# ansonb/RECON

Measured on AMD Instinct MI355X. Metric: edges aggregated/sec (GAT fwd+bwd) on synthetic KG-context graphs, higher is better.
Workload: dtype f32

## Files before the change

### recon_amd/csrc/gat_atp.hip

```cpp
#include <math.h>
#include <stdlib.h>
#include "recon_common.h"

#include <type_traits>

namespace recon {
namespace {

constexpr int kBlock = 256;

__device__ __forceinline__ int xcd_block(int b, int nb) {
    const int q = nb >> 3, r = nb & 7, x = b & 7, i = b >> 3;
    return (x < r ? x * (q + 1) : r * (q + 1) + (x - r) * q) + i;
}
template <int VEC, bool B16>
__device__ __forceinline__ void load_in(float (&r)[VEC], const float* base, int64_t e) {
    if constexpr (!B16) {
        load_vec<VEC>(r, base + e);
    } else {
        const uint16_t* b = reinterpret_cast<const uint16_t*>(base) + e;
        if constexpr (VEC == 4) {
            const uint2 t = *reinterpret_cast<const uint2*>(b);
            r[0] = __builtin_bit_cast(float, t.x << 16); r[1] = __builtin_bit_cast(float, t.x & 0xffff0000u);
            r[2] = __builtin_bit_cast(float, t.y << 16); r[3] = __builtin_bit_cast(float, t.y & 0xffff0000u);
// ... 45 lines not shown
        float t = 0.f;
#pragma unroll
        for (int g = 0; g < 16; ++g) t += red[g][c];
        u[static_cast<int64_t>(h) * W + w] = t;
    }
    if (aux) {
        __syncthreads();
        red[grp][c] = mx;
        __syncthreads();
        if (threadIdx.x < 64) {
            float m = 0.f;
#pragma unroll
            for (int g = 0; g < 16; ++g) m = fmaxf(m, red[g][threadIdx.x]);
#pragma unroll
            for (int off = 32; off > 0; off >>= 1) m = fmaxf(m, __shfl_xor(m, off, 64));
            const int b = blockIdx.y * gridDim.x + blockIdx.x;
            if (threadIdx.x == 0) aux[hx2_blkmax_word(b)] = __builtin_bit_cast(uint32_t, m);
        }
        const int nblk = gridDim.x * gridDim.y, b = blockIdx.y * gridDim.x + blockIdx.x;
        const int total = static_cast<int>(kHx2AuxBytes / 4) - kHx2QuantityWords;
        const int per_b = (total + nblk - 1) / nblk;
        for (int i = b * per_b + threadIdx.x; i < min(total, (b + 1) * per_b); i += 1024) aux[kHx2QuantityWords + i] = 0u;
    }
}

__global__ void __launch_bounds__(256) k_score_vec_bwd(const float* __restrict__ a, const float* __restrict__ a2,
                                                       const float* __restrict__ gu, int32_t D, int32_t W, float* __restrict__ ga,
                                                       float* __restrict__ ga2, uint32_t* __restrict__ rezero, int32_t rezero_words) {
    __shared__ float red[256];
    const int d = blockIdx.x, h = blockIdx.y;
    if (rezero && d == 0 && h == 0)
        for (int i = threadIdx.x; i < rezero_words; i += 256) rezero[i] = 0u;
    const int64_t row = (static_cast<int64_t>(h) * D + d) * W;
    const float a2v = a2[h * D + d];
    float s = 0.f;
    for (int w = threadIdx.x; w < W; w += 256) {
        const float g = gu[static_cast<int64_t>(h) * W + w];
        s = fmaf(a[row + w], g, s);
        if (ga) ga[row + w] += a2v * g;
    }
    red[threadIdx.x] = s;
    __syncthreads();
    for (int off = 128; off > 0; off >>= 1) {
        if (threadIdx.x < off) red[threadIdx.x] += red[threadIdx.x + off];
        __syncthreads();
    }
    if (threadIdx.x == 0 && ga2) ga2[h * D + d] = red[0];
}

__global__ void __launch_bounds__(256) k_atp_weights_finish(const float* __restrict__ partial, int32_t splits, int32_t W, int32_t D, int32_t H,
                                                            const float* __restrict__ a, const float* __restrict__ a2,
                                                            const float* __restrict__ gu, float* __restrict__ ga, float* __restrict__ ga2,
                                                            uint32_t* __restrict__ rezero, int32_t rezero_words) {
    __shared__ float tile[32][33];
    if (rezero && blockIdx.x == 0)
        for (int i = threadIdx.x; i < rezero_words; i += 256) rezero[i] = 0u;
    const int tw = (W + 31) / 32, td = (D + 31) / 32, ntile = tw * td * H;
    if (static_cast<int>(blockIdx.x) < ntile) {
        const int b = blockIdx.x, h = b / (td * tw), m0 = ((b / td) % tw) * 32, n0 = (b % td) * 32;
        const int tx = threadIdx.x & 31, ty = threadIdx.x >> 5;
        const int64_t MN = static_cast<int64_t>(W) * D;
        const float* pz = partial + static_cast<int64_t>(h) * splits * MN;
        float acc[4] = {0.f, 0.f, 0.f, 0.f};
        int64_t off[4];
        bool ok[4];
#pragma unroll
        for (int i = 0; i < 4; ++i) {
            const int m = m0 + ty + 8 * i, n = n0 + tx;
            ok[i] = m < W && n < D;
            off[i] = ok[i] ? static_cast<int64_t>(m) * D + n : 0;
        }
        for (int z = 0; z < splits; ++z) {
#pragma unroll
            for (int i = 0; i < 4; ++i) acc[i] += pz[z * MN + off[i]];
        }
#pragma unroll
        for (int i = 0; i < 4; ++i) tile[ty + 8 * i][tx] = ok[i] ? acc[i] : 0.f;
        __syncthreads();
#pragma unroll
        for (int i = 0; i < 4; ++i) {
            const int n = n0 + ty + 8 * i, m = m0 + tx;
            if (m < W && n < D)
                ga[(static_cast<int64_t>(h) * D + n) * W + m] = fmaf(a2[h * D + n], gu[static_cast<int64_t>(h) * W + m], tile[tx][ty + 8 * i]);
        }
    } else if (ga2) {
        const int lane = threadIdx.x & 63, wave = threadIdx.x >> 6;
        const int r0 = (static_cast<int>(blockIdx.x) - ntile) * 8 + wave * 2;
#pragma unroll
        for (int i = 0; i < 2; ++i) {
            const int r = r0 + i;
            if (r >= H * D) break;
            const int h = r / D;
            float sum = 0.f;
            for (int w = 4 * lane; w < W; w += 256) {
                const float4 av = *reinterpret_cast<const float4*>(a + static_cast<int64_t>(r) * W + w);
                const float4 gv = *reinterpret_cast<const float4*>(gu + static_cast<int64_t>(h) * W + w);
                sum = fmaf(av.x, gv.x, fmaf(av.y, gv.y, fmaf(av.z, gv.z, fmaf(av.w, gv.w, sum))));
            }
#pragma unroll
            for (int off = 32; off > 0; off >>= 1) sum += __shfl_xor(sum, off, 64);
            if (lane == 0) ga2[r] = sum;
        }
    }
}

__global__ void __launch_bounds__(256) k_elu_grad_q(const float* __restrict__ gy, int32_t ld_gy, const float* __restrict__ y,
                                                    int32_t ld_y, int32_t N, int32_t H, int32_t D, int32_t concat,
                                                    float* __restrict__ gh, float* __restrict__ q, uint16_t* __restrict__ ghp,
                                                    int64_t ld_p, int64_t plane_p, int32_t f16x2, const Hx2Scale gsc,
                                                    float* __restrict__ row_inv, int64_t row_inv_ld, uint32_t* __restrict__ amax_q,
                                                    const int32_t* __restrict__ row_node) {
    constexpr int IPW = 4;
    const int lane = threadIdx.x & 63;
    const int item0 = (blockIdx.x * 4 + (threadIdx.x >> 6)) * IPW;
    const int total = N * H;
    if (item0 >= total) return;
    const bool v4 = ((D | ld_gy | ld_y) & 3) == 0;
    if (v4 && D <= 256) {
        const int c = 4 * lane;
        const bool cok = c < D;
        const int cc = cok ? c : 0;
        float4 g4[IPW], y4[IPW];
#pragma unroll
        for (int j = 0; j < IPW; ++j) {
            const int it = min(item0 + j, total - 1);
            const int node = it / H, h = it % H;
            g4[j] = *reinterpret_cast<const float4*>(gy + static_cast<int64_t>(row_node ? row_node[node] : node) * ld_gy + h * D + cc);
            y4[j] = *reinterpret_cast<const float4*>(y + static_cast<int64_t>(node) * ld_y + h * D + cc);
        }
        const float gs_t = (f16x2 && !row_inv) ? hx2_scale_wave(gsc) : 1.f;
        float ov[IPW][4], pv[IPW], rmx[IPW];
#pragma unroll
        for (int j = 0; j < IPW; ++j) {
            const float gv[4] = {g4[j].x, g4[j].y, g4[j].z, g4[j].w}, yv[4] = {y4[j].x, y4[j].y, y4[j].z, y4[j].w};
            float part = 0.f, mx = 0.f;
#pragma unroll
// ... 1770 lines not shown
    const int n = blockIdx.x * (kBlock / 64) + __builtin_amdgcn_readfirstlane(threadIdx.x >> 6);
    if (n >= N) return;
    const int r = node_row[n];
    float* o = out + static_cast<int64_t>(n) * ld_out;
    const float* in = rows + static_cast<int64_t>(r < 0 ? 0 : r) * ld_rows;
    if (vec4) {
        for (int c = 4 * lane; c < width; c += 256) {
            const float4 v = r >= 0 ? *reinterpret_cast<const float4*>(in + c) : make_float4(0.f, 0.f, 0.f, 0.f);
            *reinterpret_cast<float4*>(o + c) = v;
        }
    } else {
        for (int c = lane; c < width; c += 64) o[c] = r >= 0 ? in[c] : 0.f;
    }
}
}
extern "C" int recon_rows_expand(const float* rows, int32_t ld_rows, const int32_t* node_row, int32_t N, int32_t width, float* out, int32_t ld_out,
                                 recon_stream_t stream) {
    if (N < 0 || width < 0 || ld_rows < width || ld_out < width || (N > 0 && (!node_row || !out)) || (N > 0 && width > 0 && !rows)) return RECON_ERR_INVALID;
    if (N == 0 || width == 0) return RECON_OK;
    const int vec4 = ((width | ld_rows | ld_out) & 3) == 0 && !((reinterpret_cast<uintptr_t>(rows) | reinterpret_cast<uintptr_t>(out)) & 15);
    hipLaunchKernelGGL(k_rows_expand, dim3(static_cast<unsigned>(ceil_div64(N, kBlock / 64))), dim3(kBlock), 0, as_stream(stream), rows, ld_rows, node_row, N, width, out,
                       ld_out, vec4);
    RECON_CHECK_LAUNCH();
    return RECON_OK;
}

extern "C" int recon_gat_atp_fwd(const recon_graph* g, const recon_gat_atp_args* a, recon_stream_t stream) {
    int rc = recon_gat_atp_scores(g, a, stream);
    if (rc != RECON_OK) return rc;
    rc = recon_gat_atp_aggregate(g, a, stream);
    if (rc != RECON_OK) return rc;
    return recon_gat_atp_project(g, a, stream);
}

extern "C" int recon_gat_atp_bwd_gee_bf16_supported(int32_t F, int32_t R, int32_t D, int32_t H) {
    recon::AtpShape s;
    if (!recon_gat_atp_bf16_io_supported(F, R, D, H) || !recon::atp_shape(F, R, H, &s)) return 0;
    const size_t lds_k2 = static_cast<size_t>(H) * (F + R) * sizeof(float) + (kBlock / 64) * 512;
    const bool lring = s.vec == 4 && s.kr == 1 && lds_k2 + (kBlock / 64) * kK2LdsRingBytes <= 64 * 1024 && cfg_char(CFG_K2_LDS_RING) != '0';
    return (s.ht >= H && lring) ? 1 : 0;
}

extern "C" size_t recon_gat_atp_bwd_split_bytes(int32_t N, int32_t D, int32_t H) {
    if (N <= 0 || D <= 0 || H <= 0) return 256;
    return align_up(static_cast<size_t>(3) * N * bx3_kp(H * D) * 2, 256);
}

extern "C" size_t recon_gat_atp_bwd_partial_floats(int32_t N, int32_t E, int32_t F, int32_t R, int32_t D, int32_t H) {
    const int64_t W = 2LL * F + R;
    int s1 = gemm_pick_split_k(static_cast<int32_t>(W), D, N, H);
    const int s2 = bx3_kmajor_splits(N, bx3_kmajor_split_k(static_cast<int32_t>(W), D, N, H));
    if (s2 > s1) s1 = s2;
    size_t need = static_cast<size_t>(s1) * H * D * W;
    (void)E; (void)F; (void)R;
    return need > 0 ? need : 1;
}

constexpr int kSkinnySlices = 1024;
constexpr size_t kSkinnySrcLdsMax = 32 * 1024;
static int skinny_rpb(int64_t rows) {
    const int rpb = static_cast<int>(ceil_div64(rows, kSkinnySlices));
    return rpb < 32 ? 32 : rpb;
}
extern "C" size_t recon_gat_atp_bwd_partial2_floats(int32_t N, int32_t E, int32_t F, int32_t R, int32_t D, int32_t H) {
    (void)N; (void)E; (void)D; (void)H;
    const size_t mx = static_cast<size_t>(F > R ? F : R);
    return static_cast<size_t>(3) * kSkinnySlices * 16 * mx;
}

extern "C" int recon_gat_atp_bwd(const recon_graph* g, const recon_gat_atp_bwd_args* b, recon_stream_t stream) {
    return recon_gat_atp_bwd_phase(g, b, RECON_ATP_BWD_ALL, stream);
}

extern "C" int recon_gat_atp_bwd_phase(const recon_graph* g, const recon_gat_atp_bwd_args* b, int32_t phases, recon_stream_t stream) {
    if (!b) return RECON_ERR_INVALID;
    const recon_gat_atp_args* a = &b->fwd;
    int rc = check_atp(g, a);
    if (rc != RECON_OK) return rc;
    if (!recon_gat_atp_supported(a->N, a->E, a->F, a->R, a->D, a->H)) return RECON_ERR_UNSUPPORTED;
    if (!a->Z || !a->Zk || !b->grad_out || !b->g_V || !b->gxd || !b->Gs || !b->g_u || !b->partial || !b->partial2 || !b->q) return RECON_ERR_INVALID;
    if (a->E > 0 && (!a->sigma || !b->g_sigma || !b->Gxs)) return RECON_ERR_INVALID;
    const bool hx2 = atp_hx2(a);
    if ((a->concat || atp_rows(g, a).row_node) && !b->g_h && !hx2) return RECON_ERR_INVALID;
    if (hx2 && (!b->gh_split || (reinterpret_cast<uintptr_t>(b->gh_split) & 15) || (b->ld_gout & 3))) return RECON_ERR_INVALID;
    if (b->ld_gout < a->H * a->D) return RECON_ERR_INVALID;
    if (a->N == 0) return RECON_OK;
    hipStream_t st = as_stream(stream);
    const int32_t N = a->N, E = a->E, F = a->F, R = a->R, D = a->D, H = a->H, W = 2 * F + R;
    const AtpRows rw = atp_rows(g, a);
    const int32_t NR = rw.n;
    const int64_t HD = 1LL * H * D;
    AtpShape s;
    atp_shape(F, R, H, &s);
    const size_t lds_u = static_cast<size_t>(H) * (F + R) * sizeof(float);
    if (lds_u > 60 * 1024) return RECON_ERR_UNSUPPORTED;
    const size_t lds_k2 = lds_u + (kBlock / 64) * 512;

    const float* gh = b->grad_out;
    int32_t ld_gh = b->ld_gout;
    const int64_t ld_ghp = bx3_kp(static_cast<int32_t>(HD));
    const bool gh_planes = hx2 || (b->gh_split && a->a_split && !(reinterpret_cast<uintptr_t>(b->gh_split) & 15) && (D % 8) == 0 &&
                                   ((b->ld_gout | a->ld_out) & 3) == 0);
    uint16_t* ghp = gh_planes ? static_cast<uint16_t*>(b->gh_split) : nullptr;
    const int64_t ldi = (static_cast<int64_t>(NR) + 7) / 8 * 8;
    const size_t inv_off = align_up(static_cast<size_t>(2) * N * bx3_kp(static_cast<int32_t>(HD)) * 2, 256);
    const bool row_scaled = hx2 && D <= 256 && ((a->ld_out | b->ld_gout) & 3) == 0 && cfg_char(CFG_ATP_ROW_SCALE) != '0' &&
                            inv_off + static_cast<size_t>(H) * ldi * sizeof(float) <= recon_gat_atp_bwd_split_bytes(N, D, H);
// ... 110 lines not shown
                nb_total = 0;
                for (int i = 0; i < 3; ++i) {
                    sj[i] = SkinnyJob{nullptr, nullptr, nullptr, nullptr, 0, 0, 0, 0, 1, 0};
                    rj[i] = SkinnyRedJob{nullptr, nullptr, 0, 0, 0, 0, 0, 1, 0};
                    if (i >= count) continue;
                    const Prod& q = pr[i];
                    if (q.rows <= 0) {
                        for (int j = 0; j < q.nj; ++j) (void)hipMemsetAsync(q.out + (j % q.P) * q.S1 + (j / q.P) * q.S2, 0, sizeof(float) * q.K, st);
                        continue;
                    }
                    const int rpb = skinny_rpb(q.rows);
                    const int nb = static_cast<int>(ceil_div64(q.rows, rpb));
                    float* part = b->partial2 + i * third;
                    sj[i] = SkinnyJob{q.G, q.X, q.gather, part, q.ldg, q.nj, q.rows, q.K, rpb, nb};
                    rj[i] = SkinnyRedJob{part, q.out, q.S1, q.S2, nb, q.nj, q.K, q.P, static_cast<int32_t>(ceil_div64(1LL * q.nj * q.K, 16))};
                    if (q.nj > nj_max) nj_max = q.nj;
                    nb_total += nb; nr_total += rj[i].nblocks;
                }
                if (share) { launch_src(); if (nb_total == 0) return; }
                else {
                    if (nb_total == 0) return;
                    const dim3 gp(static_cast<unsigned>(nb_total));
                    if (a->io_bf16) {
                        if (nj_max <= 8) hipLaunchKernelGGL((k_skinny_tn_partial<8, true>), gp, dim3(256), 0, st, sj[0], sj[1], sj[2]);
                        else hipLaunchKernelGGL((k_skinny_tn_partial<16, true>), gp, dim3(256), 0, st, sj[0], sj[1], sj[2]);
                    } else if (nj_max <= 8) hipLaunchKernelGGL((k_skinny_tn_partial<8>), gp, dim3(256), 0, st, sj[0], sj[1], sj[2]);
                    else hipLaunchKernelGGL((k_skinny_tn_partial<16>), gp, dim3(256), 0, st, sj[0], sj[1], sj[2]);
                }
                hipLaunchKernelGGL(k_skinny_reduce, dim3(static_cast<unsigned>(nr_total)), dim3(1024), 0, st, rj[0], rj[1], rj[2]);
            };
            if (H <= 8) {
                const Prod pr[3] = {{b->Gs, 2 * H, H, a->x, rw.row_node, NR, F, H, W, 0, b->g_u},
                                    {b->Gs + H, 2 * H, H, a->x, nullptr, N, F, H, W, 0, b->g_u + F},
                                    {b->g_sigma, H, H, a->edge_embed, ee_gather, E, R, H, W, 0, b->g_u + 2 * F}};
                run_jobs(pr, 3);
            } else {
                for (int j = 0; j < 2 * H; ++j) {
                    const Prod one = {b->Gs + j, 2 * H, 1, a->x, j < H ? rw.row_node : nullptr, j < H ? NR : N, F, 1, W, 0,
                                      b->g_u + static_cast<int64_t>(j % H) * W + (j / H) * F};
                    run_jobs(&one, 1);
                }
                for (int h0 = 0; h0 < H; h0 += 16) {
                    const int nh = H - h0 < 16 ? H - h0 : 16;
                    const Prod one = {b->g_sigma + h0, H, nh, a->edge_embed, ee_gather, E, R, nh, W, 0, b->g_u + static_cast<int64_t>(h0) * W + 2 * F};
                    run_jobs(&one, 1);
                }
            }
        }
        RECON_CHECK_LAUNCH();
    }
    }
    if (b->g_a || b->g_a_2) {
        if (!b->g_a) return RECON_ERR_INVALID;
        if (phases & RECON_ATP_BWD_WEIGHTS) {
            OperandDesc A = plain_operand(a->V, static_cast<int64_t>(H) * W);
            OperandDesc B = plain_operand(gh, ld_gh);
            OutputDesc C = plain_output(b->g_a, W);
            GemmBatch bw = bt;
            bw.a_bs = W; bw.b_bs = D; bw.c_bs = static_cast<int64_t>(D) * W; bw.c_transpose = 1;
            const int64_t ldv = static_cast<int64_t>(H) * W;
            if (hx2) {
                const int sk = bx3_kmajor_splits(NR, bx3_kmajor_split_k(W, D, NR, H));
                rc = gemm_hx2_kmajor_batched(W, D, NR, a->V, 2LL * W, W, 2LL * NR * W, b->gh_split, 2LL * D, D, 2LL * NR * D,
                                             H, sk, b->partial, static_cast<const char*>(a->aux) + kHx2ZeroPageOffset, atp_scale_v(a), atp_scale_g(a), st,
                                             atp_dst_shared(a), row_inv, ldi);
                if (rc == RECON_OK && (phases & RECON_ATP_BWD_EARLY_SUM)) rc = splitk_reduce(b->partial, sk, W, D, C, bw.c_bs, H, 0, true, st);
            } else if (gh_planes && bx3_kmajor_supported(a->V, ldv, W, ld_ghp, D, W, D)) {
                const int sk = bx3_kmajor_splits(NR, bx3_kmajor_split_k(W, D, NR, H));
                rc = gemm_bx3_kmajor_batched(W, D, NR, a->V, ldv, W, b->gh_split, ld_ghp, static_cast<int64_t>(NR) * ld_ghp, D, H, sk, b->partial, st);
                if (rc == RECON_OK) rc = splitk_reduce(b->partial, sk, W, D, C, bw.c_bs, H, 0, true, st);
            } else {
                const int sk = gemm_pick_split_k(W, D, NR, H);
                rc = gemm_f32_batched(W, D, NR, A, false, B, false, C, bw, sk, b->partial, st);
            }
            if (rc != RECON_OK) return rc;
        }
        if ((phases & RECON_ATP_BWD_FINISH) && hx2 && !(phases & RECON_ATP_BWD_EARLY_SUM)) {
            const int sk = bx3_kmajor_splits(NR, bx3_kmajor_split_k(W, D, NR, H));
            const int ntile = static_cast<int>(ceil_div64(W, 32) * ceil_div64(D, 32)) * H;
            hipLaunchKernelGGL(k_atp_weights_finish, dim3(static_cast<unsigned>(ntile + ceil_div64(1LL * H * D, 8))), dim3(256), 0, st, b->partial, sk, W,
                               D, H, a->a, a->a_2, b->g_u, b->g_a, b->g_a_2, atp_q(a, 3), kHx2QuantityWords);
        } else if (phases & RECON_ATP_BWD_FINISH)
        hipLaunchKernelGGL(k_score_vec_bwd, dim3(static_cast<unsigned>(D), static_cast<unsigned>(H)), dim3(256), 0, st, a->a, a->a_2, b->g_u,
                           D, W, b->g_a, b->g_a_2, atp_hx2(a) ? atp_q(a, 3) : nullptr, kHx2QuantityWords);
        RECON_CHECK_LAUNCH();
    } else if ((phases & RECON_ATP_BWD_FINISH) && atp_hx2(a)) {
        if (hipMemsetAsync(atp_q(a, 3), 0, sizeof(uint32_t) * kHx2QuantityWords, st) != hipSuccess) return RECON_ERR_LAUNCH;
    }
    return RECON_OK;
}
```

### recon_amd/csrc/gemm_hx2.hip

```cpp
#include <stdlib.h>
#include "gemm_tile16.h"

namespace recon {
namespace {

constexpr int T = 2;

struct Hx2Args {
    const _Float16* Ap; const _Float16* Bp;
    int64_t a_plane, a_row, a_bs;
    int64_t b_plane, b_row, b_bs;
    OutputDesc C;
    int64_t c_bs;
    int32_t M, N, K;
    int32_t epilogue, c_vec4, xcd_remap, c_plain;
    int32_t a_shared_k;
    Hx2Scale sa, sb;
    const float* row_inv; int64_t row_inv_bs;
    int32_t a_span_bytes;
};

struct Hx2Terms {
    using V = f16x8;
    static constexpr int T = 2, NP = 3;
// ... 198 lines not shown
#pragma unroll
        for (int g = 0; g < (TN + 1) / 2; ++g) {
            if (2 * g + 2 < TN) read_pair(2 * g + 2, b[(g + 1) & 1]);
            __builtin_amdgcn_sched_barrier(0);
            if (2 * g + 1 < TN) products<Hx2Terms, 2>(acc, af, b[g & 1], 2 * g);
            else products<Hx2Terms, 1>(acc, af, b[g & 1], 2 * g);
            __builtin_amdgcn_sched_barrier(0);
            if (g == 0) {
                dma_b(kt + 1, (kt + 1) & 1);
                load_a(anext2, kt + 2);
                __builtin_amdgcn_sched_barrier(0);
            }
        }
    };

    dma_b(0, 0);
    load_a(araw[0], 0);
    load_a(araw[1], 1);
    const float ia = hx2_inv(hx2_scale_wave(p.sa)), ib = hx2_inv(hx2_scale_wave(p.sb));
    int kt = 0;
#pragma unroll 1
    for (; kt + 3 <= KT; kt += 3) {
        step(kt, araw[0], araw[2]);
        step(kt + 1, araw[1], araw[0]);
        step(kt + 2, araw[2], araw[1]);
    }
    if (kt < KT) step(kt, araw[0], araw[2]);
    if (kt + 1 < KT) step(kt + 1, araw[1], araw[0]);
    (void)Kp;
    dma_wait<0>();
    float rsc[2][4];
#pragma unroll
    for (int i = 0; i < 2; ++i)
#pragma unroll
        for (int r = 0; r < 4; ++r)
            rsc[i][r] = (p.row_inv ? p.row_inv[bz * p.row_inv_bs + min(m0 + mb + 16 * i + 4 * lq + r, p.M - 1)] : 1.f) * (ia * ib);
    if (p.c_plain) {
        if (p.epilogue == GEMM_EPI_ELU) hx2_store_plain<GEMM_EPI_ELU>(acc, p.C.base + bz * p.c_bs, p.C.S1, p.M, p.N, m0, n0, mb, li, lq, rsc);
        else hx2_store_plain<GEMM_EPI_NONE>(acc, p.C.base + bz * p.c_bs, p.C.S1, p.M, p.N, m0, n0, mb, li, lq, rsc);
    } else {
        store_permuted<true>(acc, p.C, p.C.base + bz * p.c_bs, p.M, p.N, m0, n0, mb, li, lq, p.epilogue, p.c_vec4, rsc);
    }
}

struct Hx2KmArgs {
    const _Float16* Ap; const _Float16* Bp; const _Float16* zeros;
    int64_t lda, ldb, a_plane, b_plane, a_bs, b_bs;
    float* partial;
    int32_t M, N, K, k_per_split, nsplit;
    int32_t m_ld, n_ld;
    int32_t a_shared_m;
    Hx2Scale sa, sb;
    const float* k_inv; int64_t k_inv_bs;
};

constexpr int KA_PIECES = T * (KA_PLANE / 1024), KA_DMA = KA_PIECES / 4;
constexpr int KB_PIECES = T * (KB_PLANE / 1024), KB_DMA = (KB_PIECES + 3) / 4;

template <int OCC, bool KSC>
__global__ void __launch_bounds__(NT, OCC) k_gemm_hx2_kmajor(const Hx2KmArgs p) {
    __shared__ __attribute__((aligned(16))) unsigned char S[T * KA_PLANE + T * KB_PLANE];
    unsigned char* const As = S;
    unsigned char* const Bs = S + T * KA_PLANE;
    const int t = threadIdx.x, lane = t & 63;
    const int wid = __builtin_amdgcn_readfirstlane(t >> 6);
    const TileId tile = xcd_tile(1);
    const int m0 = tile.y * BM, n0 = tile.x * BN;
    const int bz = tile.z / p.nsplit, zs = tile.z % p.nsplit;
    const int k_begin = zs * p.k_per_split, k_end = min(p.K, k_begin + p.k_per_split);

    int a_k[KA_DMA];
    int64_t a_col[KA_DMA];
#pragma unroll
    for (int i = 0; i < KA_DMA; ++i) {
        const int pc = 4 * i + wid, s = 64 * (pc & 7) + lane, k = s >> 4, phys = s & 15;
        a_k[i] = k;
        a_col[i] = min(m0 + 16 * ((phys >> 1) ^ ka_h(k)) + 8 * (phys & 1), p.m_ld - 8);
        if (a_col[i] >= p.a_shared_m) a_col[i] += bz * p.a_bs;
    }
    int b_k[KB_DMA], b_col[KB_DMA];
#pragma unroll
    for (int i = 0; i < KB_DMA; ++i) {
        const int pc = min(4 * i + wid, KB_PIECES - 1);
        const int s = 64 * (pc % (KB_PIECES / T)) + lane, k = s / KB_SLOTS, phys = s % KB_SLOTS;
        int slot = phys - ((k & 8) ? 2 : 0);
        if (slot < 0 || slot >= 26) slot = 0;
        b_k[i] = k;
        b_col[i] = min(n0 + 8 * slot, p.n_ld - 8);
    }
    const _Float16* abase = p.Ap;
    const _Float16* bbase = p.Bp + bz * p.b_bs;
    const _Float16* zlane = p.zeros + 8 * lane;
    auto dma = [&](int k0) {
#pragma unroll
        for (int i = 0; i < KA_DMA; ++i) {
            const int pc = 4 * i + wid, k = k0 + a_k[i];
            const _Float16* q = k < k_end ? abase + (pc >> 3) * p.a_plane + static_cast<int64_t>(k) * p.lda + a_col[i] : zlane;
            __builtin_amdgcn_global_load_lds(reinterpret_cast<const void*>(q),
                                             (__attribute__((address_space(3))) void*)(As + (pc >> 3) * KA_PLANE + 1024 * (pc & 7)), 16, 0, 0);
        }
#pragma unroll
        for (int i = 0; i < KB_DMA; ++i)
            if (4 * i + wid < KB_PIECES) {
                const int pc = 4 * i + wid, pl = pc / (KB_PIECES / T), k = k0 + b_k[i];
                const _Float16* q = k < k_end ? bbase + pl * p.b_plane + static_cast<int64_t>(k) * p.ldb + b_col[i] : zlane;
                __builtin_amdgcn_global_load_lds(reinterpret_cast<const void*>(q),
                                                 (__attribute__((address_space(3))) void*)(Bs + pl * KB_PLANE + 1024 * (pc % (KB_PIECES / T))), 16, 0, 0);
            }
    };

    f32x4 acc[2][TN];
#pragma unroll
// ... 7 lines not shown
    bool b_rot[2];
#pragma unroll
    for (int hh = 0; hh < 2; ++hh) {
        const int k = 8 * g + 4 * hh + (ip >> 2);
#pragma unroll
        for (int i = 0; i < 2; ++i) a_off[i][hh] = k * 256 + (((2 * wid + i) ^ ka_h(k)) << 5) + ((ip & 3) << 3);
        b_row[hh] = k * (KB_SLOTS * 16) + (((ip & 3) & 1) << 3);
        b_rot[hh] = (k & 8) != 0;
    }
    auto b_off = [&](int j, int hh) { return b_row[hh] + (2 * j + ((ip & 3) >> 1) + (b_rot[hh] ? 2 : 0)) * 16; };
    float4 kin[2];
    float sg = 1.f;
    auto load_kinv = [&](int k0) {
        if constexpr (KSC) {
            const float* q = p.k_inv + bz * p.k_inv_bs + min(k0 + 8 * g, ((p.K + 7) & ~7) - 8);
            kin[0] = *reinterpret_cast<const float4*>(q);
            kin[1] = *reinterpret_cast<const float4*>(q + 4);
        }
    };
    auto mma_tile = [&]() {
        f16x8 a[2][T];
#pragma unroll
        for (int i = 0; i < 2; ++i)
#pragma unroll
            for (int q = 0; q < T; ++q) a[i][q] = tr_frag<f16x8>(As + q * KA_PLANE, a_off[i][0], a_off[i][1]);
        if constexpr (KSC) {
            const float f[8] = {kin[0].x, kin[0].y, kin[0].z, kin[0].w, kin[1].x, kin[1].y, kin[1].z, kin[1].w};
            f16x8 kf;
#pragma unroll
            for (int e = 0; e < 8; ++e) kf[e] = static_cast<_Float16>(fminf(f[e] * sg, 1.f));
#pragma unroll
            for (int i = 0; i < 2; ++i)
#pragma unroll
                for (int q = 0; q < T; ++q) a[i][q] = a[i][q] * kf;
        }
        mma_pairs<Hx2Terms>(acc, a, [&](int j, f16x8 (&dst)[T]) {
            const int o0 = b_off(j, 0), o1 = b_off(j, 1);
#pragma unroll
            for (int q = 0; q < T; ++q) dst[q] = tr_frag<f16x8>(Bs + q * KB_PLANE, o0, o1);
        });
    };

    if (k_begin < k_end) { dma(k_begin); load_kinv(k_begin); }
    const float ia = hx2_inv(hx2_scale_wave(p.sa));
    sg = hx2_scale_wave(p.sb);
    const float ib = hx2_inv(sg);
    for (int k0 = k_begin; k0 < k_end; k0 += BK) {
        asm volatile("s_waitcnt vmcnt(0)" ::: "memory");
        __syncthreads();
        mma_tile();
        __syncthreads();
        if (k0 + BK < k_end) { dma(k0 + BK); load_kinv(k0 + BK); }
    }
    float* base = p.partial + static_cast<int64_t>(tile.z) * p.M * p.N;
    const __amdgpu_buffer_rsrc_t rsrc = __builtin_amdgcn_make_buffer_rsrc(base, 0, p.M * p.N * 4, 0x00020000);
    const float sc = ia * ib;
#pragma unroll
    for (int i = 0; i < 2; ++i)
#pragma unroll
        for (int r = 0; r < 4; ++r) {
            const int row = m0 + mb + 16 * i + 4 * g + r;
            const int rowoff = row < p.M ? row * p.N : 0x1ffffff0;
#pragma unroll
            for (int j = 0; j < TN; ++j) {
                const int col = n0 + 16 * j + ip;
                const int off = col < p.N ? (rowoff + col) * 4 : 0x7ffffff0;
                __builtin_amdgcn_raw_buffer_store_b32(__builtin_bit_cast(uint32_t, acc[i][j][r] * sc), rsrc, off, 0, 0);
            }
        }
}

template <bool TRANS>
__global__ void __launch_bounds__(256) k_hx2_split_planes(const float* __restrict__ src, int64_t ld, int64_t src_bs, int32_t rows, int32_t K,
                                                          int32_t Kp, _Float16* __restrict__ dst, int64_t plane, int64_t dst_bs, const Hx2Scale sc) {
    const int64_t idx = static_cast<int64_t>(blockIdx.x) * 256 + threadIdx.x;
    const int kq = static_cast<int>(idx % (Kp / 8));
    const int r = static_cast<int>(idx / (Kp / 8));
    if (r >= rows) return;
    const float s = hx2_scale(sc);
    const float* sp = src + blockIdx.y * src_bs;
    float v[8];
#pragma unroll
    for (int j = 0; j < 8; ++j) {
        const int k = 8 * kq + j;
        v[j] = k < K ? (TRANS ? sp[static_cast<int64_t>(k) * ld + r] : sp[static_cast<int64_t>(r) * ld + k]) : 0.f;
    }
    uint32_t lo[4], hi[4];
#pragma unroll
    for (int j = 0; j < 4; ++j) hx2_split2(v[2 * j] * s, v[2 * j + 1] * s, lo[j], hi[j]);
    _Float16* d = dst + blockIdx.y * dst_bs + static_cast<int64_t>(r) * Kp + 8 * kq;
    *reinterpret_cast<u32x4*>(d) = u32x4{lo[0], lo[1], lo[2], lo[3]};
    *reinterpret_cast<u32x4*>(d + plane) = u32x4{hi[0], hi[1], hi[2], hi[3]};
}

__global__ void __launch_bounds__(256) k_hx2_split_both(const Hx2SplitBoth p) { hx2_split_both_block(p, blockIdx.x, blockIdx.y, blockIdx.z); }

template <int NTHREADS>
__global__ void __launch_bounds__(NTHREADS) k_hx2_amax(const float* __restrict__ src, int64_t rows, int32_t cols, int64_t ld, uint32_t* __restrict__ slot) {
    float m = 0.f;
    const int64_t stride = static_cast<int64_t>(gridDim.x) * NTHREADS;
    if (ld == cols && !(reinterpret_cast<uintptr_t>(src) & 15)) {
        const int64_t n = rows * cols, n4 = n >> 2;
        const float4* s4 = reinterpret_cast<const float4*>(src);
        int64_t i = static_cast<int64_t>(blockIdx.x) * NTHREADS + threadIdx.x;
        for (; i + 3 * stride < n4; i += 4 * stride) {
            const float4 v0 = s4[i], v1 = s4[i + stride], v2 = s4[i + 2 * stride], v3 = s4[i + 3 * stride];
            const float a = fmaxf(fmaxf(fabsf(v0.x), fabsf(v0.y)), fmaxf(fabsf(v0.z), fabsf(v0.w)));
            const float b = fmaxf(fmaxf(fabsf(v1.x), fabsf(v1.y)), fmaxf(fabsf(v1.z), fabsf(v1.w)));
            const float c = fmaxf(fmaxf(fabsf(v2.x), fabsf(v2.y)), fmaxf(fabsf(v2.z), fabsf(v2.w)));
// ... 71 lines not shown

bool hx2_supported(const void* Ap, int64_t a_plane, int64_t a_row, int64_t a_bs, int32_t K) {
    if (K <= 0 || (K & 7)) return false;
    return !((reinterpret_cast<uintptr_t>(Ap) & 15) || (a_plane & 7) || (a_row & 7) || (a_bs & 7));
}

int gemm_hx2_batched(int32_t M, int32_t N, int32_t K, const void* Ap, int64_t a_plane, int64_t a_row, int64_t a_bs, const void* Bplanes,
                     const OutputDesc& C, const GemmBatch& bt, const Hx2Scale& sa, const Hx2Scale& sb, hipStream_t st, int32_t a_shared_k,
                     const float* row_inv, int64_t row_inv_bs) {
    if (M < 0 || N < 0 || K < 0 || bt.batch < 0) return RECON_ERR_INVALID;
    if (M == 0 || N == 0 || bt.batch == 0) return RECON_OK;
    if (!Ap || !Bplanes || !C.base) return RECON_ERR_INVALID;
    if (!hx2_supported(Ap, a_plane, a_row, a_bs, K) || bt.c_transpose || bt.batch > 65535 || (reinterpret_cast<uintptr_t>(Bplanes) & 15))
        return RECON_ERR_UNSUPPORTED;
    Hx2Args a;
    a.Ap = static_cast<const _Float16*>(Ap); a.a_plane = a_plane; a.a_row = a_row; a.a_bs = a_bs;
    const int32_t Kp = hx2_kp(K);
    a.Bp = static_cast<const _Float16*>(Bplanes);
    a.b_row = Kp;
    a.b_bs = static_cast<int64_t>(N) * Kp;
    a.b_plane = a.b_bs * bt.batch;
    if (T * a.b_plane >= (1LL << 31)) return RECON_ERR_UNSUPPORTED;
    a.C = C; a.c_bs = bt.c_bs; a.M = M; a.N = N; a.K = K; a.epilogue = bt.epilogue;
    a.c_vec4 = c_vec4_ok(C, N, bt.c_bs) ? 1 : 0;
    a.xcd_remap = 1;
    if (a_shared_k < 0 || (a_shared_k & 7) || (a_shared_k && a_bs * bt.batch >= (1LL << 31))) return RECON_ERR_INVALID;
    a.a_shared_k = a_shared_k;
    a.c_plain = (a.c_vec4 && !C.scatter && C.P >= M && C.Dseg >= N && (static_cast<int64_t>(M) * C.S1 + N) * 4 < (1LL << 31)) ? 1 : 0;
    a.sa = sa; a.sb = sb;
    a.row_inv = row_inv; a.row_inv_bs = row_inv_bs;
    if (row_inv && sa.p0) return RECON_ERR_INVALID;
    const bool wide = K >= 1024 && ceil_div64(M, 256) * ceil_div64(N, BN) * bt.batch >= 256;
    const dim3 grid(static_cast<unsigned>(ceil_div64(N, BN)), static_cast<unsigned>(ceil_div64(M, wide ? 256 : BM)), static_cast<unsigned>(bt.batch));
    const int64_t a_span = ((T - 1) * a_plane + (bt.batch - 1) * a_bs + static_cast<int64_t>(M - 1) * a_row + hx2_kp(K) + 8) * 2;
    a.a_span_bytes = (a_plane >= 0 && a_bs >= 0 && a_row >= 0 && a_span < (1LL << 31) - 64) ? static_cast<int32_t>(a_span) : 0;
    const bool ring = !wide && a.a_span_bytes > 0 && cfg_char(CFG_HX2_RING) != '0';
    if (wide) hipLaunchKernelGGL((k_gemm_hx2<8>), grid, dim3(512), 0, st, a);
    else if (ring) hipLaunchKernelGGL((k_gemm_hx2_r3<4>), grid, dim3(NT), 0, st, a);
    else hipLaunchKernelGGL((k_gemm_hx2<4>), grid, dim3(NT), 0, st, a);
    if (hipGetLastError() != hipSuccess) return RECON_ERR_LAUNCH;
    return RECON_OK;
}

bool hx2_kmajor_supported(const void* Ap, int64_t lda, int64_t a_plane, int64_t a_bs, const void* Bp, int64_t ldb, int64_t b_plane,
                          int64_t b_bs, int32_t M, int32_t N) {
    const int64_t m_ld = (static_cast<int64_t>(M) + 7) / 8 * 8, n_ld = (static_cast<int64_t>(N) + 7) / 8 * 8;
    if (M < 1 || N < 1 || ((lda | a_plane | a_bs | ldb | b_plane | b_bs) & 7) || m_ld > lda || n_ld > ldb) return false;
    if (((M & 7) && a_bs != 0) || ((N & 7) && b_bs != 0)) return false;
    return !((reinterpret_cast<uintptr_t>(Ap) | reinterpret_cast<uintptr_t>(Bp)) & 15);
}

int gemm_hx2_kmajor_batched(int32_t M, int32_t N, int32_t K, const void* Ap, int64_t lda, int64_t a_plane, int64_t a_bs, const void* Bp,
                            int64_t ldb, int64_t b_plane, int64_t b_bs, int32_t batch, int32_t split_k, float* partial, const void* zeros,
                            const Hx2Scale& sa, const Hx2Scale& sb, hipStream_t st, int32_t a_shared_m, const float* k_inv, int64_t k_inv_bs) {
    if (M < 0 || N < 0 || K < 0 || batch < 0 || split_k < 1) return RECON_ERR_INVALID;
    if (M == 0 || N == 0 || batch == 0) return RECON_OK;
    if (!Ap || !Bp || !partial || !zeros || (reinterpret_cast<uintptr_t>(zeros) & 15)) return RECON_ERR_INVALID;
    if (!hx2_kmajor_supported(Ap, lda, a_plane, a_bs, Bp, ldb, b_plane, b_bs, M, N)) return RECON_ERR_UNSUPPORTED;
    Hx2KmArgs a;
    a.Ap = static_cast<const _Float16*>(Ap); a.Bp = static_cast<const _Float16*>(Bp); a.zeros = static_cast<const _Float16*>(zeros);
    a.lda = lda; a.ldb = ldb; a.a_plane = a_plane; a.b_plane = b_plane; a.a_bs = a_bs; a.b_bs = b_bs;
    a.partial = partial; a.M = M; a.N = N; a.K = K;
    a.m_ld = (M + 7) / 8 * 8; a.n_ld = (N + 7) / 8 * 8;
    const SplitK sp = splitk_plan(K, split_k);
    a.k_per_split = sp.k_per_split;
    a.nsplit = sp.nsplit;
    if (a.nsplit != split_k) return RECON_ERR_INVALID;
    if (static_cast<int64_t>(batch) * split_k > 65535) return RECON_ERR_UNSUPPORTED;
    a.sa = sa; a.sb = sb;
    if (a_shared_m < 0 || (a_shared_m & 7)) return RECON_ERR_UNSUPPORTED;
    a.a_shared_m = a_shared_m;
    const dim3 grid(static_cast<unsigned>(ceil_div64(N, BN)), static_cast<unsigned>(ceil_div64(M, BM)), static_cast<unsigned>(batch * split_k));
    a.k_inv = k_inv; a.k_inv_bs = k_inv_bs;
    if (k_inv && ((k_inv_bs & 3) || k_inv_bs < ((K + 7) & ~7) || (reinterpret_cast<uintptr_t>(k_inv) & 15))) return RECON_ERR_UNSUPPORTED;
    if (k_inv) hipLaunchKernelGGL((k_gemm_hx2_kmajor<2, true>), grid, dim3(NT), 0, st, a);
    else hipLaunchKernelGGL((k_gemm_hx2_kmajor<2, false>), grid, dim3(NT), 0, st, a);
    if (hipGetLastError() != hipSuccess) return RECON_ERR_LAUNCH;
    return RECON_OK;
}

}

static constexpr size_t kHdr = (recon::kHx2AuxBytes + 255) / 256 * 256;
extern "C" size_t recon_hx2_aux_bytes(void) { return recon::kHx2AuxBytes; }
static size_t hx2_planes_bytes(int64_t rows, int32_t K) { return align_up(static_cast<size_t>(2) * rows * recon::hx2_kp(K) * 2, 256); }

extern "C" size_t recon_sgemm_hx2_workspace_bytes(int32_t M, int32_t N, int32_t K) {
    if (M <= 0 || N <= 0 || K <= 0) return kHdr;
    return kHdr + hx2_planes_bytes(M, K) + hx2_planes_bytes(N, K);
}

extern "C" int recon_sgemm_hx2(int32_t M, int32_t N, int32_t K, const float* A, int32_t lda, const float* B, int32_t ldb, float* C_,
                               int32_t ldc, void* workspace, recon_stream_t stream) {
    using namespace recon;
    if (M < 0 || N < 0 || K < 0) return RECON_ERR_INVALID;
    if (M == 0 || N == 0) return RECON_OK;
    if (!A || !B || !C_ || !workspace || (reinterpret_cast<uintptr_t>(workspace) & 255)) return RECON_ERR_INVALID;
    if (K & 7) return RECON_ERR_UNSUPPORTED;
    hipStream_t st = as_stream(stream);
    char* ws = static_cast<char*>(workspace);
    uint32_t* slots = reinterpret_cast<uint32_t*>(ws);
    if (hipMemsetAsync(ws, 0, kHdr, st) != hipSuccess) return RECON_ERR_LAUNCH;
    int rc = hx2_amax(A, M, K, lda, slots + 0, st);
    if (rc == RECON_OK) rc = hx2_amax(B, N, K, ldb, slots + kHx2QuantityWords, st);
    if (rc != RECON_OK) return rc;
    const Hx2Scale sa{slots + 0, nullptr, 1.f}, sb{slots + kHx2QuantityWords, nullptr, 1.f};
    char* ap = ws + kHdr;
    char* bp = ap + hx2_planes_bytes(M, K);
    rc = hx2_split_planes(A, lda, 0, false, M, K, 1, ap, sa, st);
    if (rc == RECON_OK) rc = hx2_split_planes(B, ldb, 0, false, N, K, 1, bp, sb, st);
    if (rc != RECON_OK) return rc;
    GemmBatch bt;
    bt.batch = 1; bt.a_bs = bt.b_bs = bt.c_bs = 0; bt.epilogue = GEMM_EPI_NONE;
    const int64_t Kp = hx2_kp(K);
    return gemm_hx2_batched(M, N, K, ap, static_cast<int64_t>(M) * Kp, Kp, 0, bp, plain_output(C_, ldc), bt, sa, sb, st);
}

extern "C" int recon_sgemm_hx2_presplit(int32_t M, int32_t N, int32_t K, float* C_, int32_t ldc, void* workspace, recon_stream_t stream) {
    using namespace recon;
    if (M <= 0 || N <= 0 || K <= 0 || (K & 7) || !C_ || !workspace) return RECON_ERR_INVALID;
    char* ws = static_cast<char*>(workspace);
    uint32_t* slots = reinterpret_cast<uint32_t*>(ws);
    const Hx2Scale sa{slots + 0, nullptr, 1.f}, sb{slots + kHx2QuantityWords, nullptr, 1.f};
    char* ap = ws + kHdr;
    char* bp = ap + hx2_planes_bytes(M, K);
    GemmBatch bt;
    bt.batch = 1; bt.a_bs = bt.b_bs = bt.c_bs = 0; bt.epilogue = GEMM_EPI_NONE;
    const int64_t Kp = hx2_kp(K);
    return gemm_hx2_batched(M, N, K, ap, static_cast<int64_t>(M) * Kp, Kp, 0, bp, plain_output(C_, ldc), bt, sa, sb, as_stream(stream));
// ... 48 lines not shown
```

### recon_amd/csrc/recon_common.h

```cpp
#pragma once
#include <hip/hip_runtime.h>
#include <stdint.h>
#include "recon_hip.h"

#define RECON_CHECK_LAUNCH()                                   \
    do {                                                       \
        if (hipGetLastError() != hipSuccess) return RECON_ERR_LAUNCH; \
    } while (0)

static inline hipStream_t as_stream(recon_stream_t s) { return reinterpret_cast<hipStream_t>(s); }
static inline int64_t ceil_div64(int64_t a, int64_t b) { return (a + b - 1) / b; }
static inline size_t align_up(size_t x, size_t a) { return (x + a - 1) / a * a; }

namespace recon {

constexpr int kWave = 64;

enum CfgKey { CFG_GCN_FUSED, CFG_GCN_FUSED_BWD, CFG_GEMM_CFG, CFG_GEMM_LIN, CFG_GEMM_SPLITK, CFG_GEMM_XCD, CFG_PROP_B16, CFG_PROP_B16_YPOST,
              CFG_PROP_BWD, CFG_PROP_BWD_CHAIN, CFG_PROP_BWD_WIDE, CFG_PROP_FWD, CFG_PROP_LDS_KB, CFG_ATP_ROW_SCALE, CFG_GRAPH_SMALL, CFG_KG_NHOP,
              CFG_HX2_RING, CFG_K2_LDS_RING, CFG_K2_PERSIST, CFG_COUNT };
const char* cfg(CfgKey k);
int cfg_int(CfgKey k, int dflt);
char cfg_char(CfgKey k);
int32_t* nan_flag();
// ... 237 lines not shown
struct Hx2SplitBoth {
    const float* src; int64_t src_bs; int32_t R, C, Cp, Rp, batch, gx;
    _Float16* dst_n; _Float16* dst_t; Hx2Scale sc; uint32_t* blkmax_quantity; int32_t nblk;
};
__device__ __forceinline__ void hx2_split_both_block(const Hx2SplitBoth& p, int bx, int by, int bz) {
    typedef uint32_t u32x4_t __attribute__((ext_vector_type(4)));
    float s;
    if (p.blkmax_quantity) {
        const uint32_t bits = hx2_blkmax_wave(p.blkmax_quantity, p.nblk);
        if (bx == 0 && by == 0 && bz == 0 && threadIdx.x < kHx2Slots) p.blkmax_quantity[threadIdx.x * kHx2SlotStride] = bits;
        s = hx2_scale_of(__builtin_bit_cast(float, bits) * p.sc.mul);
    } else {
        s = hx2_scale(p.sc);
    }
    const float* sp = p.src + by * p.src_bs;
    const int64_t idx = static_cast<int64_t>(bx) * 256 + threadIdx.x;
    const int R = p.R, C_ = p.C, Cp = p.Cp, Rp = p.Rp;
    float v[8];
    _Float16* d;
    int64_t plane;
    if (bz == 0) {
        const int kq = static_cast<int>(idx % (Cp / 8)), r = static_cast<int>(idx / (Cp / 8));
        if (r >= R) return;
#pragma unroll
        for (int j = 0; j < 8; ++j) { const int k = 8 * kq + j; v[j] = k < C_ ? sp[static_cast<int64_t>(r) * C_ + k] : 0.f; }
        plane = static_cast<int64_t>(p.batch) * R * Cp;
        d = p.dst_n + (static_cast<int64_t>(by) * R + r) * Cp + 8 * kq;
    } else {
        const int c = static_cast<int>(idx % C_), kq = static_cast<int>(idx / C_);
        if (kq >= Rp / 8) return;
#pragma unroll
        for (int j = 0; j < 8; ++j) { const int k = 8 * kq + j; v[j] = k < R ? sp[static_cast<int64_t>(k) * C_ + c] : 0.f; }
        plane = static_cast<int64_t>(p.batch) * C_ * Rp;
        d = p.dst_t + (static_cast<int64_t>(by) * C_ + c) * Rp + 8 * kq;
    }
    uint32_t hi[4], lo[4];
#pragma unroll
    for (int j = 0; j < 4; ++j) hx2_split2(v[2 * j] * s, v[2 * j + 1] * s, hi[j], lo[j]);
    *reinterpret_cast<u32x4_t*>(d) = u32x4_t{hi[0], hi[1], hi[2], hi[3]};
    *reinterpret_cast<u32x4_t*>(d + plane) = u32x4_t{lo[0], lo[1], lo[2], lo[3]};
}
bool hx2_split_both_args(const float* src, int64_t src_bs, int32_t R, int32_t C_, int32_t batch, void* dst_n, void* dst_t, Hx2SplitBoth* p);
int hx2_split_planes_both(const float* src, int64_t src_bs, int32_t R, int32_t C_, int32_t batch, void* dst_n, void* dst_t, const Hx2Scale& sc,
                          hipStream_t st, uint32_t* blkmax_quantity = nullptr, int32_t nblk = 0);
bool hx2_supported(const void* Ap, int64_t a_plane, int64_t a_row, int64_t a_bs, int32_t K);
int gemm_hx2_batched(int32_t M, int32_t N, int32_t K, const void* Ap, int64_t a_plane, int64_t a_row, int64_t a_bs, const void* Bplanes,
                     const OutputDesc& C, const GemmBatch& bt, const Hx2Scale& sa, const Hx2Scale& sb, hipStream_t st, int32_t a_shared_k = 0,
                     const float* row_inv = nullptr, int64_t row_inv_bs = 0);
bool hx2_kmajor_supported(const void* Ap, int64_t lda, int64_t a_plane, int64_t a_bs, const void* Bp, int64_t ldb, int64_t b_plane,
                          int64_t b_bs, int32_t M, int32_t N);
int gemm_hx2_kmajor_batched(int32_t M, int32_t N, int32_t K, const void* Ap, int64_t lda, int64_t a_plane, int64_t a_bs, const void* Bp,
                            int64_t ldb, int64_t b_plane, int64_t b_bs, int32_t batch, int32_t split_k, float* partial, const void* zeros,
                            const Hx2Scale& sa, const Hx2Scale& sb, hipStream_t st, int32_t a_shared_m = 0, const float* k_inv = nullptr,
                            int64_t k_inv_bs = 0);
int splitk_reduce(const float* partial, int32_t splits, int32_t M, int32_t N, const OutputDesc& C, int64_t c_bs, int32_t batch,
                  int32_t epilogue, bool transpose, hipStream_t st);

}
```

Measured before the change: 82.08 million.

## Store split-K partials in native MFMA tile layout and reduce with float4 chunks

The k-major hx2 GEMM can now write its split-K partials in the accumulator's native tile order, using one contiguous 128-bit buffer store per fragment instead of scattered row-major stores. The finish kernel reads that layout with per-wave float4 loads, unrolls the split loop by eight, and writes the transposed weight gradient directly as float4 without the LDS transpose. The goal is to make both the partial writes and the reduction coalesced. In exchange, the partial buffer may need padding up to whole 128x208 tiles, and the finish kernel now depends on the GEMM's tile constants.

```diff
diff --git a/recon_amd/csrc/gat_atp.hip b/recon_amd/csrc/gat_atp.hip
--- a/recon_amd/csrc/gat_atp.hip
+++ b/recon_amd/csrc/gat_atp.hip
@@ -121,36 +121,46 @@
                                                             const float* __restrict__ a, const float* __restrict__ a2,
                                                             const float* __restrict__ gu, float* __restrict__ ga, float* __restrict__ ga2,
                                                             uint32_t* __restrict__ rezero, int32_t rezero_words) {
-    __shared__ float tile[32][33];
     if (rezero && blockIdx.x == 0)
         for (int i = threadIdx.x; i < rezero_words; i += 256) rezero[i] = 0u;
-    const int tw = (W + 31) / 32, td = (D + 31) / 32, ntile = tw * td * H;
+    const int RC = (W + 15) / 16, CC = (D + 15) / 16, nchunk = RC * CC * H, ntile = (nchunk + 3) / 4;
     if (static_cast<int>(blockIdx.x) < ntile) {
-        const int b = blockIdx.x, h = b / (td * tw), m0 = ((b / td) % tw) * 32, n0 = (b % td) * 32;
-        const int tx = threadIdx.x & 31, ty = threadIdx.x >> 5;
-        const int64_t MN = static_cast<int64_t>(W) * D;
-        const float* pz = partial + static_cast<int64_t>(h) * splits * MN;
-        float acc[4] = {0.f, 0.f, 0.f, 0.f};
-        int64_t off[4];
-        bool ok[4];
-#pragma unroll
-        for (int i = 0; i < 4; ++i) {
-            const int m = m0 + ty + 8 * i, n = n0 + tx;
-            ok[i] = m < W && n < D;
-            off[i] = ok[i] ? static_cast<int64_t>(m) * D + n : 0;
-        }
-        for (int z = 0; z < splits; ++z) {
-#pragma unroll
-            for (int i = 0; i < 4; ++i) acc[i] += pz[z * MN + off[i]];
-        }
-#pragma unroll
-        for (int i = 0; i < 4; ++i) tile[ty + 8 * i][tx] = ok[i] ? acc[i] : 0.f;
-        __syncthreads();
-#pragma unroll
-        for (int i = 0; i < 4; ++i) {
-            const int n = n0 + ty + 8 * i, m = m0 + tx;
-            if (m < W && n < D)
-                ga[(static_cast<int64_t>(h) * D + n) * W + m] = fmaf(a2[h * D + n], gu[static_cast<int64_t>(h) * W + m], tile[tx][ty + 8 * i]);
+        const int lane = threadIdx.x & 63;
+        const int c = __builtin_amdgcn_readfirstlane(static_cast<int>(blockIdx.x) * 4 + static_cast<int>(threadIdx.x >> 6));
+        if (c >= nchunk) return;
+        const int h = c / (RC * CC), cc = (c / RC) % CC, rc = c % RC;
+        const int MT = (W + kHx2KmTileM - 1) / kHx2KmTileM, NTL = (D + kHx2KmTileN - 1) / kHx2KmTileN;
+        const int mt = rc >> 3, wi = rc & 7, nt = cc / 13, j = cc % 13;
+        const int64_t image = static_cast<int64_t>(MT) * NTL * (kHx2KmTileM * kHx2KmTileN);
+        const float* q = partial + static_cast<int64_t>(h) * splits * image + ((static_cast<int64_t>(mt * NTL + nt) * 8 + wi) * 13 + j) * 256 + 4 * lane;
+        auto ld = [&](int z) { return *reinterpret_cast<const float4*>(q + z * image); };
+        float4 s = {0.f, 0.f, 0.f, 0.f};
+        auto add = [&](const float4& v) { s.x += v.x; s.y += v.y; s.z += v.z; s.w += v.w; };
+        int z = 0;
+        for (; z + 8 <= splits; z += 8) {
+            float4 v[8];
+#pragma unroll
+            for (int k = 0; k < 8; ++k) v[k] = ld(z + k);
+#pragma unroll
+            for (int k = 0; k < 8; ++k) add(v[k]);
+        }
+        if (z + 4 <= splits) {
+            float4 v[4];
+#pragma unroll
+            for (int k = 0; k < 4; ++k) v[k] = ld(z + k);
+#pragma unroll
+            for (int k = 0; k < 4; ++k) add(v[k]);
+            z += 4;
+        }
+        for (; z < splits; ++z) add(ld(z));
+        const int n = nt * kHx2KmTileN + 16 * j + (lane & 15), m = 16 * rc + 4 * (lane >> 4);
+        if (n < D && m < W) {
+            const float a2v = a2[h * D + n];
+            const float4 g = *reinterpret_cast<const float4*>(gu + static_cast<int64_t>(h) * W + m);
+            const float4 o = {fmaf(a2v, g.x, s.x), fmaf(a2v, g.y, s.y), fmaf(a2v, g.z, s.z), fmaf(a2v, g.w, s.w)};
+            float* dst = ga + (static_cast<int64_t>(h) * D + n) * W + m;
+            if (!(reinterpret_cast<uintptr_t>(ga) & 15)) *reinterpret_cast<float4*>(dst) = o;
+            else { dst[0] = o.x; dst[1] = o.y; dst[2] = o.z; dst[3] = o.w; }
         }
     } else if (ga2) {
         const int lane = threadIdx.x & 63, wave = threadIdx.x >> 6;
@@ -2027,7 +2037,11 @@
     const int s2 = bx3_kmajor_splits(N, bx3_kmajor_split_k(static_cast<int32_t>(W), D, N, H));
     if (s2 > s1) s1 = s2;
     size_t need = static_cast<size_t>(s1) * H * D * W;
-    (void)E; (void)F; (void)R;
+    if (atp_hx2_shape(F, R, D, H)) {
+        const size_t native = static_cast<size_t>(s2) * H * hx2_kmajor_native_floats(static_cast<int32_t>(W), D);
+        if (native > need) need = native;
+    }
+    (void)E;
     return need > 0 ? need : 1;
 }
 
@@ -2244,6 +2258,7 @@
     }
     if (b->g_a || b->g_a_2) {
         if (!b->g_a) return RECON_ERR_INVALID;
+        const bool native = hx2 && !(phases & RECON_ATP_BWD_EARLY_SUM);
         if (phases & RECON_ATP_BWD_WEIGHTS) {
             OperandDesc A = plain_operand(a->V, static_cast<int64_t>(H) * W);
             OperandDesc B = plain_operand(gh, ld_gh);
@@ -2255,7 +2270,7 @@
                 const int sk = bx3_kmajor_splits(NR, bx3_kmajor_split_k(W, D, NR, H));
                 rc = gemm_hx2_kmajor_batched(W, D, NR, a->V, 2LL * W, W, 2LL * NR * W, b->gh_split, 2LL * D, D, 2LL * NR * D,
                                              H, sk, b->partial, static_cast<const char*>(a->aux) + kHx2ZeroPageOffset, atp_scale_v(a), atp_scale_g(a), st,
-                                             atp_dst_shared(a), row_inv, ldi);
+                                             atp_dst_shared(a), row_inv, ldi, native);
                 if (rc == RECON_OK && (phases & RECON_ATP_BWD_EARLY_SUM)) rc = splitk_reduce(b->partial, sk, W, D, C, bw.c_bs, H, 0, true, st);
             } else if (gh_planes && bx3_kmajor_supported(a->V, ldv, W, ld_ghp, D, W, D)) {
                 const int sk = bx3_kmajor_splits(NR, bx3_kmajor_split_k(W, D, NR, H));
@@ -2267,9 +2282,9 @@
             }
             if (rc != RECON_OK) return rc;
         }
-        if ((phases & RECON_ATP_BWD_FINISH) && hx2 && !(phases & RECON_ATP_BWD_EARLY_SUM)) {
+        if ((phases & RECON_ATP_BWD_FINISH) && native) {
             const int sk = bx3_kmajor_splits(NR, bx3_kmajor_split_k(W, D, NR, H));
-            const int ntile = static_cast<int>(ceil_div64(W, 32) * ceil_div64(D, 32)) * H;
+            const int ntile = static_cast<int>(ceil_div64(ceil_div64(W, 16) * ceil_div64(D, 16) * H, 4));
             hipLaunchKernelGGL(k_atp_weights_finish, dim3(static_cast<unsigned>(ntile + ceil_div64(1LL * H * D, 8))), dim3(256), 0, st, b->partial, sk, W,
                                D, H, a->a, a->a_2, b->g_u, b->g_a, b->g_a_2, atp_q(a, 3), kHx2QuantityWords);
         } else if (phases & RECON_ATP_BWD_FINISH)
diff --git a/recon_amd/csrc/gemm_hx2.hip b/recon_amd/csrc/gemm_hx2.hip
--- a/recon_amd/csrc/gemm_hx2.hip
+++ b/recon_amd/csrc/gemm_hx2.hip
@@ -274,12 +274,14 @@
     int32_t a_shared_m;
     Hx2Scale sa, sb;
     const float* k_inv; int64_t k_inv_bs;
+    int32_t tile_native;
 };
+static_assert(BM == kHx2KmTileM && BN == kHx2KmTileN && BM == 4 * 32 && BN == TN * 16, "recon_common.h names this tile to the layout's readers");
 
 constexpr int KA_PIECES = T * (KA_PLANE / 1024), KA_DMA = KA_PIECES / 4;
 constexpr int KB_PIECES = T * (KB_PLANE / 1024), KB_DMA = (KB_PIECES + 3) / 4;
 
-template <int OCC, bool KSC>
+template <int OCC, bool KSC, bool NATIVE>
 __global__ void __launch_bounds__(NT, OCC) k_gemm_hx2_kmajor(const Hx2KmArgs p) {
     __shared__ __attribute__((aligned(16))) unsigned char S[T * KA_PLANE + T * KB_PLANE];
     unsigned char* const As = S;
@@ -393,9 +395,22 @@
         __syncthreads();
         if (k0 + BK < k_end) { dma(k0 + BK); load_kinv(k0 + BK); }
     }
+    const float sc = ia * ib;
+    if constexpr (NATIVE) {
+        const int64_t chunk0 = ((static_cast<int64_t>(tile.z) * gridDim.y + tile.y) * gridDim.x + tile.x) * (4 * 2 * TN) + wid * (2 * TN);
+        const __amdgpu_buffer_rsrc_t win = __builtin_amdgcn_make_buffer_rsrc(p.partial + chunk0 * 256, 0, 2 * TN * 1024, 0x00020000);
+        const int loff = 16 * (ip + 16 * g);
+#pragma unroll
+        for (int i = 0; i < 2; ++i) {
+            if (m0 + mb + 16 * i >= p.M) break;
+#pragma unroll
+            for (int j = 0; j < TN; ++j)
+                __builtin_amdgcn_raw_buffer_store_b128(__builtin_bit_cast(u32x4, acc[i][j] * sc), win, loff + (i * TN + j) * 1024, 0, 0);
+        }
+        return;
+    }
     float* base = p.partial + static_cast<int64_t>(tile.z) * p.M * p.N;
     const __amdgpu_buffer_rsrc_t rsrc = __builtin_amdgcn_make_buffer_rsrc(base, 0, p.M * p.N * 4, 0x00020000);
-    const float sc = ia * ib;
 #pragma unroll
     for (int i = 0; i < 2; ++i)
 #pragma unroll
@@ -573,7 +588,8 @@
 
 int gemm_hx2_kmajor_batched(int32_t M, int32_t N, int32_t K, const void* Ap, int64_t lda, int64_t a_plane, int64_t a_bs, const void* Bp,
                             int64_t ldb, int64_t b_plane, int64_t b_bs, int32_t batch, int32_t split_k, float* partial, const void* zeros,
-                            const Hx2Scale& sa, const Hx2Scale& sb, hipStream_t st, int32_t a_shared_m, const float* k_inv, int64_t k_inv_bs) {
+                            const Hx2Scale& sa, const Hx2Scale& sb, hipStream_t st, int32_t a_shared_m, const float* k_inv, int64_t k_inv_bs,
+                            bool tile_native) {
     if (M < 0 || N < 0 || K < 0 || batch < 0 || split_k < 1) return RECON_ERR_INVALID;
     if (M == 0 || N == 0 || batch == 0) return RECON_OK;
     if (!Ap || !Bp || !partial || !zeros || (reinterpret_cast<uintptr_t>(zeros) & 15)) return RECON_ERR_INVALID;
@@ -593,9 +609,13 @@
     a.a_shared_m = a_shared_m;
     const dim3 grid(static_cast<unsigned>(ceil_div64(N, BN)), static_cast<unsigned>(ceil_div64(M, BM)), static_cast<unsigned>(batch * split_k));
     a.k_inv = k_inv; a.k_inv_bs = k_inv_bs;
+    a.tile_native = tile_native ? 1 : 0;
+    if (tile_native && (reinterpret_cast<uintptr_t>(partial) & 15)) return RECON_ERR_INVALID;
     if (k_inv && ((k_inv_bs & 3) || k_inv_bs < ((K + 7) & ~7) || (reinterpret_cast<uintptr_t>(k_inv) & 15))) return RECON_ERR_UNSUPPORTED;
-    if (k_inv) hipLaunchKernelGGL((k_gemm_hx2_kmajor<2, true>), grid, dim3(NT), 0, st, a);
-    else hipLaunchKernelGGL((k_gemm_hx2_kmajor<2, false>), grid, dim3(NT), 0, st, a);
+    if (k_inv && tile_native) hipLaunchKernelGGL((k_gemm_hx2_kmajor<2, true, true>), grid, dim3(NT), 0, st, a);
+    else if (k_inv) hipLaunchKernelGGL((k_gemm_hx2_kmajor<2, true, false>), grid, dim3(NT), 0, st, a);
+    else if (tile_native) hipLaunchKernelGGL((k_gemm_hx2_kmajor<2, false, true>), grid, dim3(NT), 0, st, a);
+    else hipLaunchKernelGGL((k_gemm_hx2_kmajor<2, false, false>), grid, dim3(NT), 0, st, a);
     if (hipGetLastError() != hipSuccess) return RECON_ERR_LAUNCH;
     return RECON_OK;
 }
diff --git a/recon_amd/csrc/recon_common.h b/recon_amd/csrc/recon_common.h
--- a/recon_amd/csrc/recon_common.h
+++ b/recon_amd/csrc/recon_common.h
@@ -313,7 +313,11 @@
 int gemm_hx2_kmajor_batched(int32_t M, int32_t N, int32_t K, const void* Ap, int64_t lda, int64_t a_plane, int64_t a_bs, const void* Bp,
                             int64_t ldb, int64_t b_plane, int64_t b_bs, int32_t batch, int32_t split_k, float* partial, const void* zeros,
                             const Hx2Scale& sa, const Hx2Scale& sb, hipStream_t st, int32_t a_shared_m = 0, const float* k_inv = nullptr,
-                            int64_t k_inv_bs = 0);
+                            int64_t k_inv_bs = 0, bool tile_native = false);
+constexpr int kHx2KmTileM = 128, kHx2KmTileN = 208;
+inline int64_t hx2_kmajor_native_floats(int32_t M, int32_t N) {
+    return ceil_div64(M, kHx2KmTileM) * ceil_div64(N, kHx2KmTileN) * (kHx2KmTileM * kHx2KmTileN);
+}
 int splitk_reduce(const float* partial, int32_t splits, int32_t M, int32_t N, const OutputDesc& C, int64_t c_bs, int32_t batch,
                   int32_t epilogue, bool transpose, hipStream_t st);
 
```

Result: no change. 81.94 million, median of 2 (-0.2%).
